# cityflow-project/CityFlow

Hardware: AMD Instinct MI355X
Metric: vehicle_steps_per_sec (higher is better)
Workload: dtype f64; 1 GPU; grid_30x30 (reference generator, --tlPlan, interval 1.0) + 3000 seeded interior flows (1 veh / 6 s each until t=240 s); single engine; running_vehicles_start=96748, running_vehicles_end=71131, lanes=11160, lane_count_hash_end=cf8592fdc74305bd, backend=hip-gfx950, layout=ring, parallelism=1 gpu

## Files before the change

### cityflow_amd/csrc/hip/cfx_ring_kernels.h

```cpp
#pragma once

#include <type_traits>

#include "cfx_kernels.h"


namespace cfxd {

struct RingCtx {
#ifndef CFX_RING_CROSS2_WAVES
#define CFX_RING_CROSS2_WAVES 5
#endif
    static constexpr int kCross2Waves = CFX_RING_CROSS2_WAVES;
    DevNet n;
    DevTables t;
    SlotArrays s;
    double2 *kin;
    double2 *kinN;
    int4 *meta;
    const int2 *blkR;
    int2 *blkW;
    int32_t *slotOf;
    const uint8_t *vState;
    const int2 *ringGeo;
// ... 87 lines not shown
    return make_int4(v.x, v.y, v.z, v.w);
}
__device__ __forceinline__ double2 ntLoad2(const double2 *p) {
    const cfx_v2d v = __builtin_nontemporal_load((const cfx_v2d *) p);
    return make_double2(v.x, v.y);
}
__device__ __forceinline__ void ntStore4(int4 *p, int4 x) {
    const cfx_v4i v = {x.x, x.y, x.z, x.w};
    __builtin_nontemporal_store(v, (cfx_v4i *) p);
}
__device__ __forceinline__ void ntStore2(double2 *p, double a, double b) {
    const cfx_v2d v = {a, b};
    __builtin_nontemporal_store(v, (cfx_v2d *) p);
}

struct RingOut {
    double2 *kinN;
    int2 *blk;
    int4 *scratch;
    MoverRec *movers;
    DevScalars *sc;
    long long *finKey;
    int32_t *finVid;
    int finCap;
    int32_t *finCount;
    __device__ __forceinline__ void park(int s, double v, double iv) const { kinN[s] = make_double2(iv, v); }
    __device__ __forceinline__ double parkedSpeed(int s) const { return kinN[s].y; }
    __device__ __forceinline__ double parkedInterSpeed(int s) const { return kinN[s].x; }
    __device__ __forceinline__ void keep(int s, double dis, double speed) const { kinN[s] = make_double2(dis, speed); }
};
constexpr int kRingIdxBits = 20;

template <bool LC>
__device__ inline void finishAction(const RingCtx &c, const RingOut &o, const cfx_vehicle_template &t, int s, int d, int ,
                                    double speed, double dis, double dlen, int nd0, double v, int blockerSlot, int idx = -1,
                                    int nNow = -1, LeaverPrefetch lp = LeaverPrefetch{false, 0.0, 0, 0, 0}, int flags = -1) {
    static_assert(!LC, "the ring layout does not run lane change");
    v = min2(v, 100);
    if (nd0 < 0) {
        const bool lastRoad = flags >= 0 ? (flags & 2) != 0 : isLastRoad(c, d, c.s.route[s]);
        if (!lastRoad) v = min2(v, noCollisionSpeed(0, 1, speed, t.max_neg_acc, dlen - dis, c.interval, t.min_gap));
    }
    v = max2(v, speed - t.max_neg_acc * c.interval);
    double deltaDis;
    if (v < 0) {
        deltaDis = 0.5 * speed * speed / t.max_neg_acc;
        v = 0;
    } else {
        deltaDis = (speed + v) * c.interval / 2;
    }
    double ndis = deltaDis + dis;
    int newDrv = -1;
    if (ndis > dlen) {
        if (!lp.valid) {
            lp.nextLen = nd0 >= 0 ? c.n.drvLength[nd0] : 0.0;
            lp.vid = c.s.vid[s];
            lp.route = c.s.route[s];
            lp.routePos = c.s.routePos[s];
        }
        ndis -= dlen;
        int drivable = nd0;
        newDrv = drivable >= 0 ? drivable : -2;
        if (drivable >= 0 && ndis > lp.nextLen) {
            int nxt = nextOf(c.n, c.t, drivable, lp.route, lp.routePos);
            for (;;) {
                ndis -= c.n.drvLength[drivable];
                drivable = nxt;
                newDrv = drivable >= 0 ? drivable : -2;
                if (drivable < 0 || !(ndis > c.n.drvLength[drivable])) break;
                nxt = nextOf(c.n, c.t, drivable, lp.route, lp.routePos);
            }
        }
    }
    const int bv = blockerSlot >= 0 ? (lp.blockerVidP2 > 0 ? lp.blockerVidP2 - 2 : c.s.vid[blockerSlot]) : -1;
    if (idx < 0) {
        const int2 geo = c.ringGeo[d];
        idx = (s - geo.x - c.head[d]) & geo.y;
        nNow = cntNow(c, d);
    }
    if (newDrv == -1) {
        if (CFX_KL_NT & 4) ntStore2(&o.kinN[s], ndis, v);
        else o.kinN[s] = make_double2(ndis, v);
        if (bv >= 0) o.blk[s] = make_int2(bv, c.step);
        if (idx == nNow - 1) {
            TailRec r;
            r.dis = ndis;
            r.speed = v;
            r.slot = s;
            r.templ = lp.templP1 > 0 ? lp.templP1 - 1 : c.meta[s].x;
            r.prevDrv = lp.prevValid ? lp.prevDrv : c.s.prevDrv[s];
            r.tag = c.step;
            c.tailW[d] = r;
        }
        return;
    }
    o.kinN[s].y = -1.0;
    atomicAdd(&o.scratch[d].x, 1);
    atomicMax(&o.scratch[d].y, idx);
    if (newDrv >= 0) {
        MoverRec r;
        r.vid = lp.vid;
        r.templ = lp.templP1 > 0 ? lp.templP1 - 1 : c.meta[s].x;
        r.route = lp.route;
        r.routePos = lp.routePos;
        r.oldDrv = d;
        r.newDrv = newDrv;
        r.blockerVid = bv;
        r.dis = ndis;
        r.speed = v;
        atomicAdd(&o.scratch[newDrv].w, 1);
        r.nextIn = atomicExch(&o.scratch[newDrv].z, s);
        o.movers[s] = r;
    } else {
        const int f = finPlace(o.finCount, o.finCap);
        if (f >= 0) {
            o.finKey[f] = ((long long) d << kRingIdxBits) | idx;
            o.finVid[f] = lp.vid;
        } else {
            o.sc->overflow = 1;
        }
    }
}

static_assert(sizeof(SpawnBatch) + sizeof(RingCtx) + sizeof(VidTable) + 256 <= 8192, "kr_admit's arguments: a few KB (the runtime takes 32 KB and more, tools/kernarg_probe.hip)");

struct RingCommit {
    int4 *scratch;
    const MoverRec *movers;
    int32_t *waitHead;
    int32_t *curPhase;
    double *remain;
    int rlTrafficLight, nMaskWords;
    DevScalars *sc;
    const long long *finKey;
    const int32_t *finVid;
    double *finTerm;
    int finCap;
    int32_t *jobCount;
    HostMirror *hostMirror;
    int32_t *finTicket;
    int nStatBlocks;
    uint8_t *vStateW;
    int32_t *slotOfW;
    int exactTimes;
    int lightsDone;
    int32_t *hostCnt;
    int32_t *finCount;
};
struct CommitOut {
    int touched, head, n, tailWritten;
    int entrants;
    TailRec tail;
};
__device__ inline void commitDrivable(const RingCtx &c, const RingCommit &k, const int d, CommitOut *out = nullptr);
__device__ inline void commitStatBlock(const RingCtx &c, const RingCommit &k, const VidTable &vt, int part);
__device__ inline int commitStatBlocks(const RingCommit &k);
__device__ inline void commitClearMasks(const RingCtx &c, const RingCommit &k, int gid, int stride);

struct RingHalo {
    int on;
    const int32_t *cutIndex;
    HaloDev h;
    HaloIO io;
    long long *activeOut;
};

__device__ inline int ringHaloGlobalPrev(const RingCtx &c, const HaloDev &h, int prevDrv) {
    if (prevDrv >= c.n.L) return h.llGlobal[prevDrv - c.n.L];
    if (prevDrv <= -2) return -prevDrv - 2;
    return -1;
}

__device__ inline void ringHaloExport(const RingCtx &c, const RingCommit &k, const RingHalo &rh, int d, int ci, const CommitOut &co) {
    const HaloDev &h = rh.h;
    const int2 geo = c.ringGeo[d];
    int head = co.touched ? co.head : c.head[d];
    int n = co.touched ? co.n : c.cnt[d];
    if (ci < h.nGhost) {
        char *blk = rh.io.send[h.ghostPeer[ci]] + h.ghostSendOff[ci];
        const int in = co.entrants;
        int m = in;
        if (m > CFX_HALO_MAX_MIGRANTS) {
            m = CFX_HALO_MAX_MIGRANTS;
            k.sc->overflow = 3;
        }
        ((int32_t *) blk)[0] = m;
        ((int32_t *) blk)[1] = 0;
        HaloMigrant *rec = (HaloMigrant *) (blk + 8);
        for (int j = 0; j < m; ++j) {
            const int s = ringSlot(geo, head, n - in + j);
            const double2 kv = c.kinN[s];
            HaloMigrant r;
            r.vid = c.s.vid[s];
            r.routePos = c.s.routePos[s];
            r.prevLL = ringHaloGlobalPrev(c, h, c.s.prevDrv[s]);
            r.pad = 0;
            r.dis = kv.x;
            r.speed = kv.y;
            rec[j] = r;
        }
        h.ghostHadEntrants[ci] = in > 0;
        if (in > 0) {
            for (int j = 0; j + 1 < n; ++j) c.slotOf[c.s.vid[ringSlot(geo, head, j)]] = -1;
            head = (head + n - 1) & geo.y;
            c.head[d] = head;
            c.cnt[d] = 1;
            atomicAdd((unsigned long long *) rh.activeOut, (unsigned long long) in);
        }
        return;
    }
    const int j = ci - h.nGhost;
    if (j < h.nImport) {
        HaloTail t;
        t.vid = -1;
        t.prevLL = -1;
        t.dis = 0.0;
        t.speed = 0.0;
        if (n > 0) {
            const int s = ringSlot(geo, head, n - 1);
            const double2 kv = c.kinN[s];
            t.vid = c.s.vid[s];
            t.prevLL = ringHaloGlobalPrev(c, h, c.s.prevDrv[s]);
            t.dis = kv.x;
            t.speed = kv.y;
        }
        *(HaloTail *) (rh.io.send[h.importPeer[j]] + h.importSendOff[j]) = t;
    }
}

__device__ inline void ringHaloWriteTail(const RingCtx &c, int lane, int slot) {
    TailRec r{};
    r.slot = -1;
    if (slot >= 0) {
        const double2 kv = c.kin[slot];
        r.dis = kv.x;
        r.speed = kv.y;
        r.slot = slot;
        r.templ = c.meta[slot].x;
        r.prevDrv = c.s.prevDrv[slot];
    }
    r.tag = c.step - 1;
    const_cast<TailRec *>(c.tailR)[lane] = r;
}

__device__ inline void ringHaloImportCut(const RingCtx &c, const HaloDev &h, const HaloIO &io, const VidTable &vt, DevScalars *sc, int i) {
    if (i < h.nImport) {
        const int l = h.importLane[i];
        const char *blk = io.recv[h.importPeer[i]] + h.importRecvOff[i];
        const int m = ((const int32_t *) blk)[0];
        if (m <= 0) return;
        const HaloMigrant *rec = (const HaloMigrant *) (blk + 8);
        const int2 geo = c.ringGeo[l];
        const int head = c.head[l], n = c.cnt[l];
        if (n + m > geo.y) {
            sc->overflow = 8;
            return;
        }
        const int road = c.n.laneRoad[l];
        int last = -1;
        for (int j = 0; j < m; ++j) {
            const HaloMigrant r = rec[j];
            const int s = ringSlot(geo, head, n + j);
            const int route = vt.route[r.vid];
            const int next = nextOf(c.n, c.t, l, route, r.routePos);
            const int base = c.t.routeStart[route], len = c.t.routeStart[route + 1] - base;
            const int onLast = (next < 0 && c.t.routeRoads[base + len - 1] == road) ? 2 : 0;
            c.s.vid[s] = r.vid;
            c.s.drv[s] = l;
            c.s.prevDrv[s] = r.prevLL >= 0 ? -(r.prevLL + 2) : -1;
            c.s.routePos[s] = r.routePos;
            c.s.route[s] = route;
            c.meta[s] = make_int4(vt.templ[r.vid], next, onLast, CFX_INT_MAX);
            c.kin[s] = make_double2(r.dis, r.speed);
            const_cast<int2 *>(c.blkR)[s] = make_int2(-1, -1);
            c.slotOf[r.vid] = s;
            vt.state[r.vid] = 1;
            last = s;
        }
        c.cnt[l] = n + m;
        atomicAdd((unsigned long long *) &sc->active, (unsigned long long) m);
        ringHaloWriteTail(c, l, last);
        return;
    }
    const int j = i - h.nImport;
    if (j < h.nGhost && !h.ghostHadEntrants[j]) {
        const int g = h.ghostLane[j];
        const HaloTail t = *(const HaloTail *) (io.recv[h.ghostPeer[j]] + h.ghostRecvOff[j]);
        const int2 geo = c.ringGeo[g];
        const int head = c.head[g], n = c.cnt[g];
        for (int q = 0; q < n; ++q) {
            const int v = c.s.vid[ringSlot(geo, head, q)];
            if (v != t.vid) c.slotOf[v] = -1;
        }
        if (t.vid < 0) {
            c.cnt[g] = 0;
            ringHaloWriteTail(c, g, -1);
            return;
        }
        int prev = -1;
        if (t.prevLL >= 0) {
            const int k = h.llLocalOfGlobal[t.prevLL];
            prev = k >= 0 ? c.n.L + k : -(t.prevLL + 2);
        }
        const int s = ringSlot(geo, head, 0);
        c.s.vid[s] = t.vid;
        c.s.drv[s] = g;
        c.s.prevDrv[s] = prev;
        c.s.routePos[s] = 0;
        c.s.route[s] = vt.route[t.vid];
        c.meta[s] = make_int4(vt.templ[t.vid], -1, 0, CFX_INT_MAX);
        c.kin[s] = make_double2(t.dis, t.speed);
        const_cast<int2 *>(c.blkR)[s] = make_int2(-1, -1);
        c.slotOf[t.vid] = s;
        c.cnt[g] = 1;
        ringHaloWriteTail(c, g, s);
    }
}

__device__ inline bool ringHaloWaitPeer(const HaloIO &io, int p, DevScalars *sc) {
    unsigned spins = 0;
    while (__hip_atomic_load(io.waitFlag[p], __ATOMIC_ACQUIRE, __HIP_MEMORY_SCOPE_SYSTEM) < io.epoch) {
        if (++spins > (1u << 22)) {
            sc->overflow = 4;
            return false;
        }
        __builtin_amdgcn_s_sleep(16);
    }
    return true;
}

struct RingHaloIn {
    int on;
    const int32_t *cutIndex;
    HaloDev h;
    HaloIO io;
    long long *activeOut;
};

__global__ void kr_halo_import(RingCtx c, HaloDev h, HaloIO io, VidTable vt, DevScalars *sc, long long *activeOut) {
    if (io.nWait > 0) {
        __shared__ int ok;
        if (threadIdx.x == 0) {
            ok = 1;
            for (int p = 0; p < io.nWait && ok; ++p) ok = ringHaloWaitPeer(io, p, sc) ? 1 : 0;
        }
        __syncthreads();
        if (!ok) return;
    }
    const int i = blockIdx.x * blockDim.x + threadIdx.x;
    if (i == 0) {
        const long long out = *activeOut;
        if (out) {
            *activeOut = 0;
            atomicAdd((unsigned long long *) &sc->active, (unsigned long long) (-out));
        }
    }
    if (i < h.nImport + h.nGhost) ringHaloImportCut(c, h, io, vt, sc, i);
}

template <bool COMMIT, int NB = kAdmitRecs, class Batch = SpawnBatchT<NB>>
__global__ __launch_bounds__(kBlock) void kr_admit(RingCtx cIn, int32_t *admitStep, int32_t *waitHead, VidTable vt, DevScalars *sc,
                                                   const Batch batch, const RingCommit k, const RingHaloIn hin) {
    constexpr bool kMem = std::is_same<Batch, SpawnBatchMem>::value;
    const int d = blockIdx.x * blockDim.x + threadIdx.x;
    const bool isLane = d < cIn.n.L, inRange = d < cIn.n.L + cIn.n.K;
    int b0 = 0, b1 = 0;
    if constexpr (kMem) {
        if ((int) blockIdx.x < batch.nLaneBlocks) {
            b0 = batch.blockOff[blockIdx.x];
            b1 = batch.blockOff[blockIdx.x + 1];
        }
    }
    TailRec committed{};
    int w = -1, n = 0, head = 0, road = 0, laneIdx = 0;
    int2 geo = make_int2(0, 0);
    int wt = 0, route = 0, nextWait = -1, fn = kFirstNextUnknown;
    uint8_t pending = 0;
    if constexpr (COMMIT) {
        const int nBody = (int) gridDim.x - commitStatBlocks(k);
        if ((int) blockIdx.x >= nBody) {
            commitStatBlock(cIn, k, vt, (int) blockIdx.x - nBody);
            return;
        }
        commitClearMasks(cIn, k, d, nBody * (int) blockDim.x);
        if (inRange) committed = cIn.tailW[d];
        if (isLane) {
            w = waitHead[d];
            if (admitStep[d] == cIn.step) w = cIn.admitRec[d].y;
            n = cIn.cnt[d];
            geo = cIn.ringGeo[d];
            head = cIn.head[d];
            road = cIn.n.laneRoad[d];
            laneIdx = cIn.n.laneIndex[d];
            if (w >= 0) {
                wt = vt.templ[w];
                route = vt.route[w];
                nextWait = vt.nextWait[w];
                pending = vt.pendingCustom[w];
                fn = vt.firstNext[w];
            }
        }
        if (inRange) {
            CommitOut co;
            commitDrivable(cIn, k, d, &co);
            if (co.touched) {
                head = co.head;
                n = co.n;
                if (co.tailWritten) committed = co.tail;
            }
        }
    }
    RingCtx c = cIn;
    if constexpr (!COMMIT) {
        if (hin.on) {
            if (d == 0) {
                const long long out = *hin.activeOut;
                if (out) {
                    *hin.activeOut = 0;
                    atomicAdd((unsigned long long *) &sc->active, (unsigned long long) (-out));
                }
            }
            const int ci = isLane ? hin.cutIndex[d] : -1;
            if (ci >= 0) {
                const int nG = hin.h.nGhost;
                const int peer = ci < nG ? hin.h.ghostPeer[ci] : hin.h.importPeer[ci - nG];
                if (hin.io.nWait == 0 || ringHaloWaitPeer(hin.io, peer, sc))
                    ringHaloImportCut(c, hin.h, hin.io, vt, sc, ci < nG ? hin.h.nImport + ci : ci - nG);
            }
        }
    }
    if constexpr (COMMIT) {
        c.step = cIn.step + 1;
        c.tailR = cIn.tailW;
        c.tailW = const_cast<TailRec *>(cIn.tailR);
        c.kin = cIn.kinN;
        c.kinN = cIn.kin;
        c.blkR = cIn.blkW;
        c.blkW = const_cast<int2 *>(cIn.blkR);
    }
    __shared__ int sAdmitted;
    __shared__ cfx_vehicle_template sT[kLdsTempl];
    __shared__ int sLane[NB];
    const cfx_vehicle_template *tv = c.t.templ;
    const int nRecs = batch.n, firstNewVid = batch.firstNewVid;
    if (threadIdx.x == 0) sAdmitted = 0;
    if constexpr (kMem) {
        for (int i = threadIdx.x; i < b1 - b0 && i < NB; i += blockDim.x) sLane[i] = batch.lane[b0 + i];
    } else {
        for (int i = threadIdx.x; i < nRecs; i += blockDim.x) sLane[i] = batch.lane[i];
    }
    auto laneOfRec = [&](int j) {
        if constexpr (kMem) return j - b0 < NB ? sLane[j - b0] : batch.lane[j];
        else return sLane[j];
    };
    const int recLo = kMem ? b0 : 0, recHi = kMem ? b1 : nRecs;
    if (c.t.nTempl <= kLdsTempl) {
        const int nd = c.t.nTempl * (int) (sizeof(cfx_vehicle_template) / sizeof(double));
        const double *src = (const double *) c.t.templ;
        double *dst = (double *) sT;
        for (int i = threadIdx.x; i < nd; i += blockDim.x) dst[i] = src[i];
        tv = sT;
    }
    if constexpr (!COMMIT) {
        if (inRange) committed = c.tailR[d];
        if (isLane) {
            w = waitHead[d];
            n = c.cnt[d];
            geo = c.ringGeo[d];
            head = c.head[d];
            road = c.n.laneRoad[d];
            laneIdx = c.n.laneIndex[d];
        }
        if (w >= 0) {
            wt = vt.templ[w];
            route = vt.route[w];
            nextWait = vt.nextWait[w];
            pending = vt.pendingCustom[w];
            fn = vt.firstNext[w];
        }
    }
    __syncthreads();
    if (nRecs > 0) {
        auto writeRows = [&](int from, int to) {
            for (int i = from + (int) threadIdx.x; i < to; i += blockDim.x) {
                const int v = firstNewVid + batch.vidOff[i];
                vt.priority[v] = batch.priority[i];
                vt.templ[v] = batch.templ[i];
                vt.route[v] = batch.route[i];
                vt.enterTime[v] = batch.enterTime;
                vt.state[v] = 0;
                vt.pendingCustom[v] = 0;
                vt.firstNext[v] = batch.firstNext[i];
            }
        };
        if constexpr (kMem) {
            writeRows(blockIdx.x == 0 ? 0 : b0, b1);
        } else {
            if (blockIdx.x == 0) writeRows(0, nRecs);
        }
        if (isLane) {
            int lo = recLo, hi = recHi;
            while (lo < hi) {
                const int mid = (lo + hi) >> 1;
                if (laneOfRec(mid) < d) lo = mid + 1;
                else hi = mid;
            }
            int headRec = -1;
            for (int j = lo; j < recHi && laneOfRec(j) == d; ++j) {
                const int pv = batch.prevWait[j], v = firstNewVid + batch.vidOff[j];
                bool becomesHead = pv < 0;
                if (pv >= firstNewVid) vt.nextWait[pv] = v;
                else if (pv >= 0) {
                    if (vt.state[pv] != 0) becomesHead = true;
                    else vt.nextWait[pv] = v;
                }
                if (becomesHead) headRec = j;
            }
            if (headRec >= 0) {
                w = firstNewVid + batch.vidOff[headRec];
                wt = batch.templ[headRec];
                route = batch.route[headRec];
                fn = batch.firstNext[headRec];
                pending = 0;
                nextWait = -1;
                waitHead[d] = w;
            }
            if (w >= 0)
                for (int j = lo; j < recHi && laneOfRec(j) == d; ++j)
                    if (batch.prevWait[j] == w) nextWait = firstNewVid + batch.vidOff[j];
        }
    }
    if (inRange) {
        TailRec now = committed;
        if (committed.tag != c.step - 1) now.slot = -1;
        if (!isLane) {
            const int k = d - c.n.L, in = c.n.llInter[k];
            const int ph = c.curPhase[in];
            if (c.gatePhase[((c.step + 1) & 1) * c.n.I + in] != ph) {
                const int flags = (c.n.phaseAvail[c.n.interAvailStart[in] + ph * c.n.interNRL[in] + c.n.llRoadLink[k]] != 0 ? 1 : 0) |
                                  (c.n.llType[k] << 1) | (c.n.llXStart[k + 1] > c.n.llXStart[k] ? 8 : 0);
                c.llGate[k] = make_int4(flags, c.n.llEndLane[k], c.n.llXStart[k], c.n.llXStart[k + 1]);
            }
            if (c.n.llLocal[k] == 0) c.gatePhase[(c.step & 1) * c.n.I + in] = ph;
        } else {
            const int lane = d;
            bool admit = w >= 0;
            if (admit && now.slot >= 0 && !(now.dis > tv[now.templ].len + tv[wt].min_gap)) admit = false;
            if (admit && n >= geo.y) {
                sc->overflow = 8;
                admit = false;
            }
            if (admit) {
                int next, onLast;
                admittedNext(c, fn, lane, road, laneIdx, route, &next, &onLast);
                const int slot = ringSlot(geo, head, n);
                const double v0 = tv[wt].initial_speed;
                c.s.vid[slot] = w;
                c.s.drv[slot] = lane;
                c.s.prevDrv[slot] = -1;
                c.s.routePos[slot] = 0;
                c.s.route[slot] = route;
                c.meta[slot] = make_int4(wt, next, pending | onLast, CFX_INT_MAX);
                c.kin[slot] = make_double2(0.0, v0);
// ... 845 lines not shown
        double *dst = (double *) sT;
        for (int i = t; i < nd; i += kListBlock) dst[i] = src[i];
        tv = sT;
        __syncthreads();
    }
    const bool valid = qv < total;
    const int lane = t & 63;
    const int slot = valid ? e.x : 0, d = e.y, idx = valid ? e.z : 0;
    KSTAMP(11, 1);
    SlotIn in;
    in.vid = 0;
    in.dis = 0.0;
    in.speed = 0.0;
    in.templIdx = 0;
    in.nd0 = -1;
    in.flags = 0;
    double2 kp = make_double2(0.0, 0.0);
    int tp = 0;
    double2 lm = make_double2(0.0, 0.0);
    int4 hop = make_int4(-2, -2, -2, -2), en = make_int4(-1, -1, -1, -1);
    if (valid) {
        const double2 kv = (CFX_KL_NT & 8) ? ntLoad2(&c.kin[slot]) : c.kin[slot];
        const int4 mv = (CFX_KL_NT & 16) ? ntLoad4(&c.meta[slot]) : c.meta[slot];
        lm = c.n.drvLM[d];
        if (d < c.n.L) {
            hop = c.n.laneLL4[d];
            en = c.n.laneEnd4[d];
        }
        if (idx > 0 && lane == 0) {
            kp = c.kin[ls];
            tp = c.meta[ls].x;
        }
        in.dis = kv.x;
        in.speed = kv.y;
        in.templIdx = mv.x;
        in.nd0 = mv.y;
        in.flags = mv.z;
        in.lastRoadFlags = mv.z;
    }
    const int slotUp = __shfl_up(slot, 1, 64);
    const double disUp = __shfl_up(in.dis, 1, 64), speedUp = __shfl_up(in.speed, 1, 64);
    const int templUp = __shfl_up(in.templIdx, 1, 64);
    if (!valid) return;
    if (lane != 0) ls = slotUp;
    in.d = d;
    in.head = idx == 0;
    in.idx = idx;
    in.nNow = e.w & 0x7fffffff;
    in.leaderSlot = idx > 0 ? ls : 0;
    in.disPrev = lane == 0 ? kp.x : disUp;
    in.speedPrev = lane == 0 ? kp.y : speedUp;
    in.templPrev = lane == 0 ? tp : templUp;
    if (in.flags & (kFlagCustom | kFlagStateGap)) {
        in.vid = c.s.vid[slot];
        c.meta[slot].z = in.flags & ~(kFlagCustom | kFlagStateGap);
    }
    in.lm = lm;
    in.hop = make_int4(-2, -2, -2, -2);
    in.endLane = -1;
    if (in.nd0 >= c.n.L) {
        in.hop = hop;
        const int ll = in.nd0 - c.n.L;
        in.endLane = hop.x == ll ? en.x : (hop.y == ll ? en.y : (hop.z == ll ? en.z : (hop.w == ll ? en.w : -1)));
    }
    in.laneAdmitted = e.w < 0;
    const RingPush push{q, jobRecs, c.n.L};
    KSTAMP(11, 2);
    actionOneRounds<GHOST>(c, o, tv, slot, in, push);
    KSTAMP(11, 3);
}


__device__ inline void ringCopySlot(const RingCtx &c, int from, int to) {
    c.s.vid[to] = c.s.vid[from];
    c.s.drv[to] = c.s.drv[from];
    c.s.prevDrv[to] = c.s.prevDrv[from];
    c.s.routePos[to] = c.s.routePos[from];
    c.s.route[to] = c.s.route[from];
    c.meta[to] = c.meta[from];
    c.blkW[to] = c.blkW[from];
    c.kinN[to] = c.kinN[from];
    c.slotOf[c.s.vid[from]] = to;
}

__device__ inline bool ringFinishStatistics(const RingCtx &c, const VidTable &vt, const RingCommit &k, int part, int nParts) {
    __shared__ long long fin[kFinLds];
    __shared__ double term[kFinLds];
    __shared__ int lastShared;
    __shared__ FinMap fm;
    DevScalars *sc = k.sc;
    const int F = finMapLoad(fm, k.finCount, k.finCap);
    const double now = c.step * c.interval;
    auto foldAdmissions = [&]() {
        const long long a = sc->admitPending[c.step & 1];
        sc->admitPending[c.step & 1] = 0;
        sc->vehicleSteps += a;
        sc->active += a;
    };
    if (k.exactTimes) {
        const bool lastBlock = exactFinishStatistics(now, vt, sc, F, [&](int i) { return k.finVid[finAt(fm, k.finCap, i)]; }, k.vStateW,
                                                     k.finTicket, part, nParts, 0, k.finCount, k.slotOfW);
        if (lastBlock && threadIdx.x == 0) foldAdmissions();
        return lastBlock;
    }
    const bool inLds = nParts == 1 && F <= kFinLds;
    const int per = (F + nParts - 1) / nParts;
    const int lo = part * per, hi = min(F, lo + per);
    for (int base = lo; base < hi; base += blockDim.x) {
        const int i = base + (int) threadIdx.x;
        const int at = i < hi ? finAt(fm, k.finCap, i) : 0;
        const long long me = i < hi ? k.finKey[at] : 0;
        int rank = 0;
        for (int cb = 0; cb < F; cb += kFinLds) {
            const int cn = min(kFinLds, F - cb);
            __syncthreads();
            for (int j = threadIdx.x; j < cn; j += blockDim.x) fin[j] = k.finKey[finAt(fm, k.finCap, cb + j)];
            __syncthreads();
            if (i < hi)
                for (int j = 0; j < cn; ++j) rank += fin[j] < me;
        }
        if (i < hi) {
            const int vid = k.finVid[at];
            const double tt = now - vt.enterTime[vid];
            k.vStateW[vid] = 2;
            k.slotOfW[vid] = -1;
            if (inLds) term[rank] = tt;
            else k.finTerm[rank] = tt;
        }
    }
    bool last = true;
    if (nParts > 1) {
        __threadfence();
        __syncthreads();
        if (threadIdx.x == 0) lastShared = atomicAdd(k.finTicket, 1) == nParts - 1;
        __syncthreads();
        last = lastShared != 0;
        if (!last) return false;
        if (threadIdx.x == 0) *k.finTicket = 0;
        __threadfence();
    }
    __syncthreads();
    const double cum = orderedSum(sc->cumulativeTravelTime, F, term, k.finTerm, inLds);
    if (threadIdx.x == 0) {
        sc->cumulativeTravelTime = cum;
        sc->vehicleSteps += sc->active;
        sc->finishedCnt += F;
        sc->active -= F;
        finCountsClear(k.finCount);
        foldAdmissions();
    }
    return last;
}

__device__ inline void commitDrivable(const RingCtx &c, const RingCommit &k, const int d, CommitOut *out) {
    const int4 sc = k.scratch[d];
    const bool admitted = d < c.n.L && c.admitStep[d] == c.step;
    if (out) {
        out->touched = 0;
        out->entrants = 0;
    }
    if (!admitted && sc.x == 0 && sc.z < 0) return;
    const int2 geo = c.ringGeo[d];
    int head = c.head[d];
    int n = c.cnt[d];
    if (admitted) {
        const int2 rec = c.admitRec[d];
        k.waitHead[d] = rec.y;
        k.vStateW[rec.x] = 1;
        n += 1;
    }
    if (sc.x > 0) {
        if (sc.y + 1 != sc.x) {
            int wr = n - 1;
            for (int r = n - 1; r >= 0; --r) {
                const int from = ringSlot(geo, head, r);
                if (c.kinN[from].y < 0.0) continue;
                if (wr != r) ringCopySlot(c, from, ringSlot(geo, head, wr));
                --wr;
            }
        }
        head = (head + sc.x) & geo.y;
        n -= sc.x;
    }
    int m = 0, tailRank = -1;
    TailRec tail{};
    for (int e = sc.z; e >= 0; e = k.movers[e].nextIn) {
        const MoverRec r = k.movers[e];
        int rank = 0;
        for (int f = sc.z; f >= 0; f = k.movers[f].nextIn) {
            if (f == e) continue;
            const double od = k.movers[f].dis;
            const bool tieBefore = od == r.dis && k.movers[f].vid < r.vid;
            rank += (od > r.dis) || tieBefore;
            if (tieBefore) k.sc->tieDrv[atomicAdd((unsigned long long *) &k.sc->tieEvents, 1ULL) & 7ULL] = d;
        }
        ++m;
        if (n + rank > geo.y) {
            k.sc->overflow = 8;
            continue;
        }
        const int slot = ringSlot(geo, head, n + rank);
        int rp = r.routePos;
        c.s.vid[slot] = r.vid;
        c.s.drv[slot] = d;
        c.s.prevDrv[slot] = r.oldDrv;
        c.s.route[slot] = r.route;
        c.blkW[slot] = make_int2(r.blockerVid, c.step);
        int next, enterLLT, onLast = 0;
        if (d < c.n.L) {
            enterLLT = CFX_INT_MAX;
            const int base = c.t.routeStart[r.route], len = c.t.routeStart[r.route + 1] - base;
            const int road = c.n.laneRoad[d], laneIdx = c.n.laneIndex[d];
            const int p0 = rp < len ? rp : len - 1, p1 = rp + 1 < len ? rp + 1 : len - 1;
            const int road0 = c.t.routeRoads[base + p0], road1 = c.t.routeRoads[base + p1];
            int row = c.t.nextStart[base + p0];
            const int row1 = c.t.nextStart[base + p1], roadLast = c.t.routeRoads[base + len - 1];
            if (rp < len && road0 != road) {
                ++rp;
                row = row1;
                if (rp < len && road1 != road) {
                    ++rp;
                    while (rp < len && c.t.routeRoads[base + rp] != road) ++rp;
                    if (rp < len) row = c.t.nextStart[base + rp];
                }
            }
            next = -1;
            if (rp < len) {
                const int ll = c.t.nextLL[row + laneIdx];
                next = ll < 0 ? -1 : c.n.L + ll;
            }
            if (next < 0 && road == roadLast) onLast = 2;
        } else {
            enterLLT = c.step;
            next = c.n.llEndLane[d - c.n.L];
        }
        c.s.routePos[slot] = rp;
        c.meta[slot] = make_int4(r.templ, next, onLast, enterLLT);
        c.kinN[slot] = make_double2(r.dis, r.speed);
        c.slotOf[r.vid] = slot;
        if (rank > tailRank) {
            tailRank = rank;
            tail.dis = r.dis;
            tail.speed = r.speed;
            tail.slot = slot;
            tail.templ = r.templ;
            tail.prevDrv = r.oldDrv;
        }
    }
    n += m;
    if (tailRank >= 0) {
        tail.tag = c.step;
        c.tailW[d] = tail;
    } else if (sc.x > 0) {
        if (n == 0) {
            tail.slot = -1;
        } else {
            const int ts = ringSlot(geo, head, n - 1);
            const double2 kt = c.kinN[ts];
            tail.dis = kt.x;
            tail.speed = kt.y;
            tail.slot = ts;
            tail.templ = c.meta[ts].x;
            tail.prevDrv = c.s.prevDrv[ts];
        }
        tail.tag = c.step;
        c.tailW[d] = tail;
    }
    if (n > geo.y) k.sc->overflow = 8;
    else if (n + min(8, (geo.y + 1) / 2) > geo.y) k.sc->ringNearFull = 1;
    c.head[d] = head;
    c.cnt[d] = n;
    if (k.hostCnt && d < c.n.L) k.hostCnt[d] = n;
    k.scratch[d] = make_int4(0, -1, -1, 0);
    if (out) {
        out->touched = 1;
        out->head = head;
        out->n = n;
        out->tailWritten = (tailRank >= 0 || sc.x > 0) ? 1 : 0;
        out->entrants = m;
        out->tail = tail;
    }
}

__device__ inline int commitStatBlocks(const RingCommit &k) { return k.nStatBlocks; }
__device__ inline void commitStatBlock(const RingCtx &c, const RingCommit &k, const VidTable &vt, int part) {
    if (part == 0 && threadIdx.x < kJobShards) k.jobCount[threadIdx.x * kJobShardStride] = 0;
    const bool last = ringFinishStatistics(c, vt, k, part, k.nStatBlocks);
    if (last && threadIdx.x == 0 && k.hostMirror) {
        k.hostMirror->sc = *k.sc;
        k.sc->actionMaxT = 0;
        k.hostMirror->slots = (int32_t) k.sc->active;
        __hip_atomic_store(&k.hostMirror->progress, ((unsigned long long) (c.step + 1) << 32) | (unsigned) k.sc->active,
                           __ATOMIC_RELAXED, __HIP_MEMORY_SCOPE_SYSTEM);
    }
}
__device__ inline void commitClearMasks(const RingCtx &c, const RingCommit &k, int gid, int stride) {
    for (int i = gid; i < k.nMaskWords; i += stride) c.interMask[i] = 0ULL;
}

__global__ __launch_bounds__(kBlock) void kr_commit(RingCtx c, RingCommit k, VidTable vt, RingHalo rh) {
    const int nBody = (int) gridDim.x - k.nStatBlocks;
    if ((int) blockIdx.x >= nBody) {
        commitStatBlock(c, k, vt, (int) blockIdx.x - nBody);
        return;
    }
    const int gid = blockIdx.x * blockDim.x + threadIdx.x;
    const int stride = nBody * blockDim.x;
    commitClearMasks(c, k, gid, stride);
    if (!k.rlTrafficLight && !k.lightsDone) passTimeAll(c.n, k.curPhase, k.remain, c.interval, gid, stride);
    const int D = c.n.L + c.n.K;
    for (int d = gid; d < D; d += stride) {
        CommitOut co;
        commitDrivable(c, k, d, &co);
        if (rh.on && d < c.n.L) {
            const int ci = rh.cutIndex[d];
            if (ci >= 0) {
                ringHaloExport(c, k, rh, d, ci, co);
                if (rh.io.nSignal > 0) {
                    const int nCut = rh.h.nGhost + rh.h.nImport;
                    __threadfence_system();
                    if (atomicAdd(rh.io.ticket, 1) == nCut - 1) {
                        __threadfence_system();
                        *rh.io.ticket = 0;
                        for (int p = 0; p < rh.io.nSignal; ++p)
                            __hip_atomic_store(rh.io.signalFlag[p], rh.io.epoch, __ATOMIC_RELEASE, __HIP_MEMORY_SCOPE_SYSTEM);
                    }
                }
            }
        }
    }
}

struct RingDense {
    int32_t *vid, *drv, *prevDrv, *blockerVid, *enterLLT, *routePos, *leaderVid;
    uint8_t *flags;
    double *dis, *speed, *gap;
};

__global__ void kr_gather(RingCtx c, const int32_t *off, RingDense out, int wantLeader) {
    const int d = blockIdx.x * blockDim.x + threadIdx.x;
    if (d >= c.n.L + c.n.K) return;
    const int n = c.cnt[d];
    if (n == 0) return;
    const int2 geo = c.ringGeo[d];
    const int head = c.head[d], o = off[d];
    for (int i = 0; i < n; ++i) {
        const int s = ringSlot(geo, head, i);
        out.vid[o + i] = c.s.vid[s];
        out.drv[o + i] = d;
        out.prevDrv[o + i] = c.s.prevDrv[s];
        out.blockerVid[o + i] = blockerVid(c, s);
        const double2 kv = c.kin[s];
        const int4 mv = c.meta[s];
        out.enterLLT[o + i] = mv.w;
        out.routePos[o + i] = c.s.routePos[s];
        out.flags[o + i] = (uint8_t) (mv.z & (kFlagCustom | kFlagStateGap));
        out.dis[o + i] = kv.x;
        out.speed[o + i] = kv.y;
        if (wantLeader) {
            double gap = 0;
            int ls;
            if (i > 0) {
                ls = ringSlot(geo, head, i - 1);
                gap = c.kin[ls].x - c.t.templ[c.meta[ls].x].len - kv.x;
            } else {
                ls = findHeadLeader(c, c.t.templ, s, d, kv.x, c.t.templ[mv.x].approach_dist, mv.y, c.n.drvLength[d], &gap).slot;
            }
            if ((mv.z & kFlagStateGap) && ls >= 0) gap = c.vGapState[c.s.vid[s]];
            out.leaderVid[o + i] = ls >= 0 ? c.s.vid[ls] : -1;
            out.gap[o + i] = gap;
        }
    }
}

__global__ void kr_scatter_in(RingCtx c, const int32_t *off, RingDense in, VidTable vt) {
    const int d = blockIdx.x * blockDim.x + threadIdx.x;
    if (d >= c.n.L + c.n.K) return;
    const int n = off[d + 1] - off[d];
    c.head[d] = 0;
    c.cnt[d] = n;
    const int2 geo = c.ringGeo[d];
    for (int i = 0; i < n; ++i) {
        const int s = geo.x + i, j = off[d] + i;
        const int v = in.vid[j];
        const int route = vt.route[v];
        c.s.vid[s] = v;
        c.s.drv[s] = d;
        c.s.prevDrv[s] = in.prevDrv[j];
        c.s.routePos[s] = in.routePos[j];
        c.s.route[s] = route;
        const_cast<int2 *>(c.blkR)[s] = make_int2(in.blockerVid[j], c.step - 1);
        c.kin[s] = make_double2(in.dis[j], in.speed[j]);
        const int nextD = nextOf(c.n, c.t, d, route, in.routePos[j]);
        c.meta[s] = make_int4(vt.templ[v], nextD, (in.flags[j] & (kFlagCustom | kFlagStateGap)) | ((nextD < 0 && isLastRoad(c, d, route)) ? 2 : 0), in.enterLLT[j]);
        c.slotOf[v] = s;
        if (i == n - 1) {
            TailRec r;
            r.dis = in.dis[j];
            r.speed = in.speed[j];
            r.slot = s;
            r.templ = vt.templ[v];
            r.prevDrv = in.prevDrv[j];
            r.tag = c.step - 1;
            const_cast<TailRec *>(c.tailR)[d] = r;
        }
    }
}

constexpr int kOffBlock = 1024;
__global__ __launch_bounds__(kOffBlock) void kr_offsets(const int32_t *in, int32_t *out, int n) {
    __shared__ int sWaveSum[kOffBlock / 64];
    __shared__ int sCarry;
    const int t = (int) threadIdx.x, lane = t & 63, wv = t >> 6;
    if (t == 0) sCarry = 0;
    __syncthreads();
    for (int base = 0; base < n; base += kOffBlock * 4) {
        const int i0 = base + t * 4;
        int v[4];
        for (int j = 0; j < 4; ++j) v[j] = i0 + j < n ? in[i0 + j] : 0;
        const int mine = v[0] + v[1] + v[2] + v[3];
        int incl = mine;
        for (int off = 1; off < 64; off <<= 1) {
            const int up = __shfl_up(incl, off, 64);
            if (lane >= off) incl += up;
        }
        if (lane == 63) sWaveSum[wv] = incl;
        __syncthreads();
        int before = sCarry + incl - mine;
        for (int i = 0; i < wv; ++i) before += sWaveSum[i];
        for (int j = 0; j < 4; ++j) {
            if (i0 + j < n) out[i0 + j] = before;
            before += v[j];
        }
        __syncthreads();
        if (t == kOffBlock - 1) sCarry = before;
        __syncthreads();
    }
}

__global__ void kr_reset(int D, int32_t *head, int32_t *cnt, int4 *scratch) {
    const int d = blockIdx.x * blockDim.x + threadIdx.x;
    if (d >= D) return;
    head[d] = 0;
    cnt[d] = 0;
    scratch[d] = make_int4(0, -1, -1, 0);
}

__global__ void kr_lane_history(RingCtx c, LaneHistDev h) { ringLaneHistory(c, h, blockIdx.x * blockDim.x + threadIdx.x); }

struct RingLaneRec {
    const double2 *kin;
    int2 geo;
    int head;
    __device__ __forceinline__ double2 operator()(int i) const { return kin[ringSlot(geo, head, i)]; }
};
__device__ __forceinline__ RingLaneRec laneRec(const RingCtx &c, int lane) { return RingLaneRec{c.kin, c.ringGeo[lane], c.head[lane]}; }

struct RingLaneVid {
    const int32_t *vid;
    int2 geo;
    int head;
    __device__ __forceinline__ int operator()(int i) const { return vid[ringSlot(geo, head, i)]; }
};
__device__ __forceinline__ RingLaneVid laneVid(const RingCtx &c, int lane) { return RingLaneVid{c.s.vid, c.ringGeo[lane], c.head[lane]}; }

__global__ void __launch_bounds__(kBlock) kr_lane_features(RingCtx c, LaneFeatOut o) {
// ... 91 lines not shown
```

Baseline: 1.996 billion vehicle-steps/s.

## Preload commit inputs and batch mover processing to overlap dependent loads

Per-drivable commit state (scratch, geometry, head, count, admission, lane road/index, wait head) is now loaded up front into a struct, with scheduling barriers so the loads are issued together. The fused kernel reuses these values instead of reloading them. Movers are gathered into a small register array (CAP, default 1) so rank comparisons and route-table lookups can be unrolled and their loads issued in batches. Mask clearing moves after the commit, and admission writes are deferred to the end. The intent is to hide global-memory latency on the commit path. The cost is extra register pressure, and the inline asm barriers restrict how the compiler can schedule the code.

Result: slower. 1.737 billion vehicle-steps/s (-13.0%).

```diff
diff --git a/cityflow_amd/csrc/hip/cfx_ring_kernels.h b/cityflow_amd/csrc/hip/cfx_ring_kernels.h
--- a/cityflow_amd/csrc/hip/cfx_ring_kernels.h
+++ b/cityflow_amd/csrc/hip/cfx_ring_kernels.h
@@ -263,7 +263,70 @@
     int entrants;
     TailRec tail;
 };
-__device__ inline void commitDrivable(const RingCtx &c, const RingCommit &k, const int d, CommitOut *out = nullptr);
+#ifndef CFX_COMMIT_INLINE
+#define CFX_COMMIT_INLINE 1
+#endif
+constexpr int kCommitInline = CFX_COMMIT_INLINE;
+struct CommitPre {
+    int4 sc;
+    int2 geo, admitRec;
+    int head, cnt, admitStep;
+    int road, laneIdx;
+    int waitHead;
+    int endLane;
+};
+__device__ __forceinline__ void awaitLoads(struct CommitPre &p);
+__device__ __forceinline__ CommitPre commitPreload(const RingCtx &c, const RingCommit &k, const int d) {
+    CommitPre p{};
+    p.admitStep = p.waitHead = p.endLane = -1;
+    p.sc = k.scratch[d];
+    if (d < c.n.L) {
+        p.geo = c.ringGeo[d];
+        p.head = c.head[d];
+        p.cnt = c.cnt[d];
+        p.admitStep = c.admitStep[d];
+        p.admitRec = c.admitRec[d];
+        p.road = c.n.laneRoad[d];
+        p.laneIdx = c.n.laneIndex[d];
+        p.waitHead = k.waitHead[d];
+        awaitLoads(p);
+    }
+    return p;
+}
+__device__ __forceinline__ void commitPreloadLink(const RingCtx &c, const RingCommit &k, const int d, CommitPre &p) {
+    if (d >= c.n.L && (p.sc.x != 0 || p.sc.z >= 0)) {
+        p.geo = c.ringGeo[d];
+        p.head = c.head[d];
+        p.cnt = c.cnt[d];
+        p.endLane = c.n.llEndLane[d - c.n.L];
+    }
+}
+__device__ __forceinline__ void awaitLoads(int &a) {
+    __builtin_amdgcn_sched_barrier(0);
+    asm volatile("" : "+v"(a));
+}
+__device__ __forceinline__ void awaitLoads(int &a, int &b) {
+    __builtin_amdgcn_sched_barrier(0);
+    asm volatile("" : "+v"(a), "+v"(b));
+}
+__device__ __forceinline__ void awaitLoads(int &a, int &b, int &c) {
+    __builtin_amdgcn_sched_barrier(0);
+    asm volatile("" : "+v"(a), "+v"(b), "+v"(c));
+}
+__device__ __forceinline__ void awaitLoads(CommitPre &p) {
+    __builtin_amdgcn_sched_barrier(0);
+    asm volatile("" : "+v"(p.sc.x), "+v"(p.sc.y), "+v"(p.sc.z), "+v"(p.geo.x), "+v"(p.geo.y), "+v"(p.head), "+v"(p.cnt), "+v"(p.admitStep),
+                 "+v"(p.admitRec.x), "+v"(p.admitRec.y), "+v"(p.road), "+v"(p.laneIdx), "+v"(p.waitHead));
+}
+template <int N>
+__device__ __forceinline__ void awaitLoads(int (&v)[N]) {
+    static_assert(N >= 1 && N <= 3, "one asm statement for all of them");
+    if constexpr (N == 1) awaitLoads(v[0]);
+    else if constexpr (N == 2) awaitLoads(v[0], v[1]);
+    else awaitLoads(v[0], v[1], v[2]);
+}
+template <int CAP = kCommitInline>
+__device__ inline void commitDrivable(const RingCtx &c, const RingCommit &k, const int d, const CommitPre &p, CommitOut *out = nullptr);
 __device__ inline void commitStatBlock(const RingCtx &c, const RingCommit &k, const VidTable &vt, int part);
 __device__ inline int commitStatBlocks(const RingCommit &k);
 __device__ inline void commitClearMasks(const RingCtx &c, const RingCommit &k, int gid, int stride);
@@ -493,16 +556,18 @@
             commitStatBlock(cIn, k, vt, (int) blockIdx.x - nBody);
             return;
         }
-        commitClearMasks(cIn, k, d, nBody * (int) blockDim.x);
-        if (inRange) committed = cIn.tailW[d];
+        CommitPre pre{};
+        if (inRange) {
+            committed = cIn.tailW[d];
+            pre = commitPreload(cIn, k, d);
+        }
         if (isLane) {
-            w = waitHead[d];
-            if (admitStep[d] == cIn.step) w = cIn.admitRec[d].y;
-            n = cIn.cnt[d];
-            geo = cIn.ringGeo[d];
-            head = cIn.head[d];
-            road = cIn.n.laneRoad[d];
-            laneIdx = cIn.n.laneIndex[d];
+            w = pre.admitStep == cIn.step ? pre.admitRec.y : pre.waitHead;
+            n = pre.cnt;
+            geo = pre.geo;
+            head = pre.head;
+            road = pre.road;
+            laneIdx = pre.laneIdx;
             if (w >= 0) {
                 wt = vt.templ[w];
                 route = vt.route[w];
@@ -513,13 +578,15 @@
         }
         if (inRange) {
             CommitOut co;
-            commitDrivable(cIn, k, d, &co);
+            commitPreloadLink(cIn, k, d, pre);
+            commitDrivable(cIn, k, d, pre, &co);
             if (co.touched) {
                 head = co.head;
                 n = co.n;
                 if (co.tailWritten) committed = co.tail;
             }
         }
+        commitClearMasks(cIn, k, d, nBody * (int) blockDim.x);
     }
     RingCtx c = cIn;
     if constexpr (!COMMIT) {
@@ -1671,23 +1738,35 @@
     return last;
 }
 
-__device__ inline void commitDrivable(const RingCtx &c, const RingCommit &k, const int d, CommitOut *out) {
-    const int4 sc = k.scratch[d];
-    const bool admitted = d < c.n.L && c.admitStep[d] == c.step;
+template <int CAP>
+__device__ inline void commitDrivable(const RingCtx &c, const RingCommit &k, const int d, const CommitPre &p, CommitOut *out) {
+    const int4 sc = p.sc;
+    const bool isLane = d < c.n.L;
+    const bool admitted = isLane && p.admitStep == c.step;
     if (out) {
         out->touched = 0;
         out->entrants = 0;
     }
     if (!admitted && sc.x == 0 && sc.z < 0) return;
-    const int2 geo = c.ringGeo[d];
-    int head = c.head[d];
-    int n = c.cnt[d];
-    if (admitted) {
-        const int2 rec = c.admitRec[d];
-        k.waitHead[d] = rec.y;
-        k.vStateW[rec.x] = 1;
-        n += 1;
-    }
+    const MoverRec *const mv = k.movers;
+    MoverRec r[CAP];
+    int e = sc.z, nPass = 0;
+    auto gather = [&]() {
+        nPass = 0;
+#pragma unroll
+        for (int i = 0; i < CAP; ++i)
+            if (e >= 0) {
+                r[i] = mv[e];
+                e = r[i].nextIn;
+                nPass = i + 1;
+            }
+    };
+    gather();
+    const bool onePass = e < 0;
+    const int2 geo = p.geo;
+    int head = p.head;
+    int n = p.cnt;
+    if (admitted) n += 1;
     if (sc.x > 0) {
         if (sc.y + 1 != sc.x) {
             int wr = n - 1;
@@ -1703,68 +1782,111 @@
     }
     int m = 0, tailRank = -1;
     TailRec tail{};
-    for (int e = sc.z; e >= 0; e = k.movers[e].nextIn) {
-        const MoverRec r = k.movers[e];
-        int rank = 0;
-        for (int f = sc.z; f >= 0; f = k.movers[f].nextIn) {
-            if (f == e) continue;
-            const double od = k.movers[f].dis;
-            const bool tieBefore = od == r.dis && k.movers[f].vid < r.vid;
-            rank += (od > r.dis) || tieBefore;
+    const int road = p.road, laneIdx = p.laneIdx;
+    while (nPass > 0) {
+        int rank[CAP];
+        auto versus = [&](int i, double od, int ovid) {
+            const bool tieBefore = od == r[i].dis && ovid < r[i].vid;
+            rank[i] += (od > r[i].dis) || tieBefore;
             if (tieBefore) k.sc->tieDrv[atomicAdd((unsigned long long *) &k.sc->tieEvents, 1ULL) & 7ULL] = d;
-        }
-        ++m;
-        if (n + rank > geo.y) {
-            k.sc->overflow = 8;
-            continue;
-        }
-        const int slot = ringSlot(geo, head, n + rank);
-        int rp = r.routePos;
-        c.s.vid[slot] = r.vid;
-        c.s.drv[slot] = d;
-        c.s.prevDrv[slot] = r.oldDrv;
-        c.s.route[slot] = r.route;
-        c.blkW[slot] = make_int2(r.blockerVid, c.step);
-        int next, enterLLT, onLast = 0;
-        if (d < c.n.L) {
-            enterLLT = CFX_INT_MAX;
-            const int base = c.t.routeStart[r.route], len = c.t.routeStart[r.route + 1] - base;
-            const int road = c.n.laneRoad[d], laneIdx = c.n.laneIndex[d];
-            const int p0 = rp < len ? rp : len - 1, p1 = rp + 1 < len ? rp + 1 : len - 1;
-            const int road0 = c.t.routeRoads[base + p0], road1 = c.t.routeRoads[base + p1];
-            int row = c.t.nextStart[base + p0];
-            const int row1 = c.t.nextStart[base + p1], roadLast = c.t.routeRoads[base + len - 1];
-            if (rp < len && road0 != road) {
-                ++rp;
-                row = row1;
-                if (rp < len && road1 != road) {
-                    ++rp;
-                    while (rp < len && c.t.routeRoads[base + rp] != road) ++rp;
-                    if (rp < len) row = c.t.nextStart[base + rp];
+        };
+#pragma unroll
+        for (int i = 0; i < CAP; ++i) rank[i] = 0;
+        if (onePass) {
+#pragma unroll
+            for (int i = 0; i < CAP; ++i)
+#pragma unroll
+                for (int j = 0; j < CAP; ++j)
+                    if (j != i && i < nPass && j < nPass) versus(i, r[j].dis, r[j].vid);
+        } else {
+            for (int f = sc.z; f >= 0;) {
+                const MoverRec o = mv[f];
+#pragma unroll
+                for (int i = 0; i < CAP; ++i)
+                    if (i < nPass && o.vid != r[i].vid) versus(i, o.dis, o.vid);
+                f = o.nextIn;
+            }
+        }
+        int rp[CAP], next[CAP], onLast[CAP];
+#pragma unroll
+        for (int i = 0; i < CAP; ++i) {
+            rp[i] = r[i].routePos;
+            next[i] = p.endLane;
+            onLast[i] = 0;
+        }
+        if (isLane) {
+            int base[CAP], len[CAP], road0[CAP], road1[CAP], row[CAP], row1[CAP], roadLast[CAP], ll[CAP];
+#pragma unroll
+            for (int i = 0; i < CAP; ++i) row[i] = 0;
+#pragma unroll
+            for (int i = 0; i < CAP; ++i)
+                if (i < nPass) {
+                    base[i] = c.t.routeStart[r[i].route];
+                    len[i] = c.t.routeStart[r[i].route + 1] - base[i];
                 }
-            }
-            next = -1;
-            if (rp < len) {
-                const int ll = c.t.nextLL[row + laneIdx];
-                next = ll < 0 ? -1 : c.n.L + ll;
-            }
-            if (next < 0 && road == roadLast) onLast = 2;
-        } else {
-            enterLLT = c.step;
-            next = c.n.llEndLane[d - c.n.L];
-        }
-        c.s.routePos[slot] = rp;
-        c.meta[slot] = make_int4(r.templ, next, onLast, enterLLT);
-        c.kinN[slot] = make_double2(r.dis, r.speed);
-        c.slotOf[r.vid] = slot;
-        if (rank > tailRank) {
-            tailRank = rank;
-            tail.dis = r.dis;
-            tail.speed = r.speed;
-            tail.slot = slot;
-            tail.templ = r.templ;
-            tail.prevDrv = r.oldDrv;
-        }
+#pragma unroll
+            for (int i = 0; i < CAP; ++i)
+                if (i < nPass) {
+                    const int p0 = rp[i] < len[i] ? rp[i] : len[i] - 1, p1 = rp[i] + 1 < len[i] ? rp[i] + 1 : len[i] - 1;
+                    road0[i] = c.t.routeRoads[base[i] + p0];
+                    road1[i] = c.t.routeRoads[base[i] + p1];
+                    row[i] = c.t.nextStart[base[i] + p0];
+                    row1[i] = c.t.nextStart[base[i] + p1];
+                    roadLast[i] = c.t.routeRoads[base[i] + len[i] - 1];
+                }
+#pragma unroll
+            for (int i = 0; i < CAP; ++i)
+                if (i < nPass && rp[i] < len[i] && road0[i] != road) {
+                    ++rp[i];
+                    row[i] = row1[i];
+                    if (rp[i] < len[i] && road1[i] != road) {
+                        ++rp[i];
+                        while (rp[i] < len[i] && c.t.routeRoads[base[i] + rp[i]] != road) ++rp[i];
+                        if (rp[i] < len[i]) row[i] = c.t.nextStart[base[i] + rp[i]];
+                    }
+                }
+            awaitLoads(row);
+#pragma unroll
+            for (int i = 0; i < CAP; ++i) {
+                ll[i] = -1;
+                if (i < nPass && rp[i] < len[i]) ll[i] = c.t.nextLL[row[i] + laneIdx];
+            }
+#pragma unroll
+            for (int i = 0; i < CAP; ++i)
+                if (i < nPass) {
+                    next[i] = ll[i] < 0 ? -1 : c.n.L + ll[i];
+                    if (next[i] < 0 && road == roadLast[i]) onLast[i] = 2;
+                }
+        }
+        const int enterLLT = isLane ? CFX_INT_MAX : c.step;
+#pragma unroll
+        for (int i = 0; i < CAP; ++i) {
+            if (i >= nPass) continue;
+            ++m;
+            if (n + rank[i] > geo.y) {
+                k.sc->overflow = 8;
+                continue;
+            }
+            const int slot = ringSlot(geo, head, n + rank[i]);
+            c.s.vid[slot] = r[i].vid;
+            c.s.drv[slot] = d;
+            c.s.prevDrv[slot] = r[i].oldDrv;
+            c.s.route[slot] = r[i].route;
+            c.blkW[slot] = make_int2(r[i].blockerVid, c.step);
+            c.s.routePos[slot] = rp[i];
+            c.meta[slot] = make_int4(r[i].templ, next[i], onLast[i], enterLLT);
+            c.kinN[slot] = make_double2(r[i].dis, r[i].speed);
+            c.slotOf[r[i].vid] = slot;
+            if (rank[i] > tailRank) {
+                tailRank = rank[i];
+                tail.dis = r[i].dis;
+                tail.speed = r[i].speed;
+                tail.slot = slot;
+                tail.templ = r[i].templ;
+                tail.prevDrv = r[i].oldDrv;
+            }
+        }
+        gather();
     }
     n += m;
     if (tailRank >= 0) {
@@ -1787,6 +1909,11 @@
     }
     if (n > geo.y) k.sc->overflow = 8;
     else if (n + min(8, (geo.y + 1) / 2) > geo.y) k.sc->ringNearFull = 1;
+    if (admitted) {
+        const int2 rec = p.admitRec;
+        k.waitHead[d] = rec.y;
+        k.vStateW[rec.x] = 1;
+    }
     c.head[d] = head;
     c.cnt[d] = n;
     if (k.hostCnt && d < c.n.L) k.hostCnt[d] = n;
@@ -1830,7 +1957,9 @@
     const int D = c.n.L + c.n.K;
     for (int d = gid; d < D; d += stride) {
         CommitOut co;
-        commitDrivable(c, k, d, &co);
+        CommitPre pre = commitPreload(c, k, d);
+        commitPreloadLink(c, k, d, pre);
+        commitDrivable(c, k, d, pre, &co);
         if (rh.on && d < c.n.L) {
             const int ci = rh.cutIndex[d];
             if (ci >= 0) {
```
